# harman097/RoboRugby

Measured on AMD Instinct MI355X. Metric: env_steps_per_sec, higher is better.
Workload: dtype f64

## Files before the change

roborugby_amd/build.py:

```python
import hashlib
import os
import re
import shutil
import subprocess

HERE = os.path.dirname(os.path.abspath(__file__))
SRC = os.path.join(HERE, "csrc", "rr_kernels.hip")
SRC_KSTEP = os.path.join(HERE, "csrc", "rr_kstep_inst.hip")
SRC_DQN = os.path.join(HERE, "csrc", "rr_dqn.hip")
HDR_KSTEP = os.path.join(HERE, "csrc", "rr_kstep.hpp")
DEPS = [SRC, SRC_KSTEP, SRC_DQN, HDR_KSTEP, os.path.join(HERE, "csrc", "rr_sim.hpp"),
        os.path.join(HERE, "csrc", "rr_extras.hpp"), os.path.join(HERE, "csrc", "rr_hive.hpp"),
        os.path.join(os.path.dirname(HERE), "include", "roborugby_amd.h")]
LIB = os.path.join(HERE, "libroborugby_amd.so")
LIB_EXACT = os.path.join(HERE, "libroborugby_amd_exact.so")
HIPCC_FLAGS = ["-O3", "--offload-arch=gfx950", "-std=c++17", "-ffp-contract=off", "-fPIC", "-shared"]


def header_config_table():
    with open(HDR_KSTEP) as f:
        text = f.read()
    parts = int(re.search(r"^#define RR_KSTEP_PARTS (\d+)$", text, re.M).group(1))
    table = re.search(r"^#else // the product library.*?^#endif", text, re.M | re.S).group(0)
    rows = [tuple(int(v) for v in m.groups()) for m in re.finditer(r"X\((\d+), (\d+), (\d+), (\d+), (\d+), (\d+), \w+, \d+, [01]\)", table)]
    if not rows or sorted({r[1] for r in rows}) != list(range(parts)):
        raise RuntimeError("csrc/rr_kstep.hpp: the configuration table does not use every part 0..RR_KSTEP_PARTS-1")
    return parts, {r[2:] for r in rows}


KSTEP_PARTS = 7
BUILT_SHAPES = {(1, 0, 1, 0), (2, 2, 4, 4), (1, 1, 1, 1)}


def find_hipcc():
    for cand in (shutil.which("hipcc"), "/opt/rocm/bin/hipcc"):
        if cand and os.path.exists(cand):
            return cand
    raise RuntimeError("hipcc not found: the MI355X library cannot be built here")


def sources_present():
    return all(os.path.exists(d) for d in DEPS)


def source_hash():
    h = hashlib.sha256(" ".join(HIPCC_FLAGS).encode())
    for d in DEPS:
        with open(d, "rb") as f:
            h.update(os.path.basename(d).encode() + b"\0" + f.read())
    return h.hexdigest()


def is_stale(exact=False):
    lib = LIB_EXACT if exact else LIB
    if not os.path.exists(lib) or not os.path.exists(lib + ".srchash"):
        return True
    with open(lib + ".srchash") as f:
        return f.read().strip() != source_hash()


def build_hip_library(force=False, verbose=False, jobs=None, exact=False):
    lib_path = LIB_EXACT if exact else LIB
    if not force and not is_stale(exact):
        return lib_path
    import tempfile
    from concurrent.futures import ThreadPoolExecutor
    if header_config_table() != (KSTEP_PARTS, BUILT_SHAPES):
        raise RuntimeError("roborugby_amd/build.py: KSTEP_PARTS / BUILT_SHAPES differ from the table in csrc/rr_kstep.hpp")
    digest = source_hash()
    hipcc = find_hipcc()
    cflags = [f for f in HIPCC_FLAGS if f != "-shared"] + (["-DRR_EXACT_TRIG=1"] if exact else [])
    jobs = jobs or int(os.environ.get("RR_BUILD_JOBS", "0")) or min(8, os.cpu_count() or 1)
    with tempfile.TemporaryDirectory(prefix="rr_build_") as tmpd:
        units = [(SRC, ["-DRR_SPLIT_BUILD"], os.path.join(tmpd, "rr_kernels.o"))]
        units += [(SRC_KSTEP, [f"-DRR_PART={k}"], os.path.join(tmpd, f"rr_kstep_{k}.o")) for k in range(KSTEP_PARTS)]
        units += [(SRC_DQN, [], os.path.join(tmpd, "rr_dqn.o"))]

        def compile_one(u):
            src, defs, obj = u
            cmd = [hipcc] + cflags + defs + ["-c", "-o", obj, src]
            if verbose:
                print(" ".join(cmd), flush=True)
            subprocess.check_call(cmd)
            return obj

        with ThreadPoolExecutor(max_workers=jobs) as ex:
            objs = list(ex.map(compile_one, units))
        tmp = lib_path + f".tmp{os.getpid()}"
        cmd = [hipcc, "--offload-arch=gfx950", "-fPIC", "-shared", "-o", tmp] + objs
        if verbose:
            print(" ".join(cmd), flush=True)
        subprocess.check_call(cmd)
    os.replace(tmp, lib_path)
    with open(lib_path + ".srchash", "w") as f:
# ... 61 lines not shown
```

roborugby_amd/csrc/rr_kernels.hip:

```cpp
#include <hip/hip_runtime.h>
#include <stdio.h>
#include <string.h>
#include <cmath>
#include <new>
#include <string>
#include <type_traits>
#include <cstdlib>

#include "../../include/roborugby_amd.h"
#include "rr_sim.hpp"
#include "rr_extras.hpp"
#include "rr_hive.hpp"
#include "rr_kstep.hpp"

using namespace rr;


#ifndef RR_ORDER_SHIFT
#define RR_ORDER_SHIFT 2
#endif
constexpr int ORDER_BINS = 1024, ORDER_THREADS = 1024;
__global__ __launch_bounds__(ORDER_THREADS) void k_order(const uint32_t *cost, uint32_t *order, int ngroups) {
    __shared__ uint32_t hist[ORDER_BINS];
    for (int i = threadIdx.x; i < ORDER_BINS; i += ORDER_THREADS) hist[i] = 0;
    __syncthreads();
    for (int g = threadIdx.x; g < ngroups; g += ORDER_THREADS) {
        uint32_t c = cost[g] >> RR_ORDER_SHIFT;
        c = c > ORDER_BINS - 1 ? ORDER_BINS - 1 : c;
        atomicAdd(&hist[ORDER_BINS - 1 - c], 1u);
    }
    __syncthreads();
    __shared__ uint32_t scan[ORDER_BINS];
    uint32_t v = hist[threadIdx.x];
    scan[threadIdx.x] = v;
    __syncthreads();
    for (int off = 1; off < ORDER_BINS; off <<= 1) {
        uint32_t add = threadIdx.x >= (unsigned)off ? scan[threadIdx.x - off] : 0u;
        __syncthreads();
        scan[threadIdx.x] += add;
        __syncthreads();
    }
    hist[threadIdx.x] = scan[threadIdx.x] - v;
    __syncthreads();
    for (int g = threadIdx.x; g < ngroups; g += ORDER_THREADS) {
        uint32_t c = cost[g] >> RR_ORDER_SHIFT;
        c = c > ORDER_BINS - 1 ? ORDER_BINS - 1 : c;
        order[atomicAdd(&hist[ORDER_BINS - 1 - c], 1u)] = (uint32_t)g;
    }
}
__global__ void k_iota(uint32_t *order, int n) {
    int i = blockIdx.x * blockDim.x + threadIdx.x;
    if (i < n) order[i] = (uint32_t)i;
}

template <class C, typename O>
__global__ __launch_bounds__(64 * WAVES_PER_BLOCK) void k_reset(SimParams<typename C::Real> sp, typename C::Store *recs,
                                                               int32_t *irecs, int n, const uint8_t *mask, int init,
                                                               O *obs, O *obs_g) {
    using R = typename C::Real;
    __shared__ Arena<C> lds[arenas_per_block<C>()];
    const int wave = threadIdx.x / C::VW;
    const int arena = blockIdx.x * arenas_per_block<C>() + wave;
    if (arena >= n || wave >= arenas_per_block<C>()) return;
    Arena<C> &A = lds[wave];
    typename C::Store *rec = recs + (size_t)arena * Arena<C>::P_STRIDE;
    int32_t *irec = irecs + (size_t)arena * Arena<C>::I_STRIDE;
    int st = 0;
    if (init) {
        const int lane = threadIdx.x & (C::VW - 1);
        R *p = reinterpret_cast<R *>(&A.p);
        int32_t *q = reinterpret_cast<int32_t *>(&A.i);
        for (int k = lane; k < Arena<C>::P_REALS; k += C::VW) p[k] = (R)0;
        for (int k = lane; k < Arena<C>::I_INTS; k += C::VW) q[k] = 0;
        RR_SYNC();
        if (lane < C::NR) robot_set_clean_lane(A, sp, lane, (R)0, (R)0, lane < C::NRH ? (R)90 : (R)-90);
        if (lane < C::NB) ball_set_clean_lane(A, lane, (R)0, (R)0, (R)0, (R)0);
        if (lane == 0) A.i.episode = -1;
        RR_SYNC();
    } else {
        load_record(A, rec, irec);
    }
    const bool doit = init || !mask || mask[arena];
    if (doit) reset_arena(A, sp, sp.arena_offset + (uint64_t)arena, (uint64_t)(uint32_t)(A.i.episode + 1), st);
    else derive(A, sp);
    if (obs && doit) observe<C, O>(A, sp, 1, -1, -1, obs + (size_t)arena * 11, st);
    if (obs_g && doit) {
        if (!observe<C, O>(A, sp, -1, -1, -1, obs_g + (size_t)arena * 11, st)) {
            for (int k = threadIdx.x & (C::VW - 1); k < 11; k += C::VW) obs_g[(size_t)arena * 11 + k] = (O)NAN;
        }
    }
    store_record(A, rec, irec);
}

template <class C, typename O>
__global__ __launch_bounds__(64 * WAVES_PER_BLOCK) void k_observe(SimParams<typename C::Real> sp, const typename C::Store *recs,
                                                                 const int32_t *irecs, int n, int team, int ridx, int bidx,
                                                                 O *obs) {
    __shared__ Arena<C> lds[arenas_per_block<C>()];
    const int wave = threadIdx.x / C::VW;
    const int arena = blockIdx.x * arenas_per_block<C>() + wave;
    if (arena >= n || wave >= arenas_per_block<C>()) return;
    Arena<C> &A = lds[wave];
    load_record(A, recs + (size_t)arena * Arena<C>::P_STRIDE, irecs + (size_t)arena * Arena<C>::I_STRIDE);
    derive(A, sp);
    int st = 0;
    if (!observe<C, O>(A, sp, team, ridx, bidx, obs + (size_t)arena * 11, st)) {
        for (int k = threadIdx.x & (C::VW - 1); k < 11; k += C::VW) obs[(size_t)arena * 11 + k] = (O)NAN;
    }
}

template <class C>
__global__ void k_set_state(typename C::Store *recs, int32_t *irecs, int n, const double *robots, const int32_t *ri,
                            const double *balls, const int32_t *step) {
    using R = typename C::Real;
    int a = blockIdx.x * blockDim.x + threadIdx.x;
    if (a >= n) return;
    typename C::Store *rec = recs + (size_t)a * Arena<C>::P_STRIDE;
    int32_t *irec = irecs + (size_t)a * Arena<C>::I_STRIDE;
    using L = RecLayout<C>;
    constexpr int NR = C::NR, NB = C::NB;
    for (int r = 0; r < NR; r++) {
        for (int f = 0; f < L::ROBOT_FIELDS; f++) rec[L::robot_field(f) + r] = (typename C::Store)robots[((size_t)a * NR + r) * L::ROBOT_FIELDS + f];
        for (int f = 0; f < 3; f++) irec[L::robot_int(f) + r] = ri[((size_t)a * NR + r) * 3 + f];
    }
    for (int b = 0; b < NB; b++)
        for (int f = 0; f < L::BALL_FIELDS; f++) rec[L::ball_field(f) + b] = (typename C::Store)balls[((size_t)a * NB + b) * L::BALL_FIELDS + f];
    irec[L::STEP] = step[a];
    irec[L::FAULT] = 0;
    irec[L::FZP] = 0;
#if RR_CARRY
    rec[L::IC] = rec[L::BCX + NB - 1]; rec[L::IC + 1] = rec[L::BCY + NB - 1];
#endif
// ... 123 lines not shown
    int a = blockIdx.x * blockDim.x + threadIdx.x;
    if (a >= n) return;
    if (record_parked<C>(irecs + (size_t)a * Arena<C>::I_STRIDE)) *flag = 1;
}
template <class C>
__global__ void k_goal_clear(int n, int32_t *gs, const uint8_t *mask) {
    int a = blockIdx.x * blockDim.x + threadIdx.x;
    if (a >= n || (mask && !mask[a])) return;
    goal_state_clear<C>(gs + (size_t)a * gs_stride<C>());
}
template <class C>
__global__ void k_goal_scores(int n, const int32_t *gs, int32_t *scores) {
    int a = blockIdx.x * blockDim.x + threadIdx.x;
    if (a >= n) return;
    for (int k = 0; k < 2; k++) scores[2 * a + k] = goal_score<C>(gs + (size_t)a * gs_stride<C>(), k);
}
template <class C, typename O>
__global__ void k_observe_kind(SimParams<typename C::Real> sp, const typename C::Store *recs, int n, int kind, int team, int ridx,
                               int bidx, O *obs, int dim, const typename C::Real *xs) {
    int a = blockIdx.x * blockDim.x + threadIdx.x;
    if (a >= n) return;
    Rec<C> q = { recs + (size_t)a * Arena<C>::P_STRIDE };
    O tmp[6 * C::NR + 4 * C::NB > 11 ? 6 * C::NR + 4 * C::NB : 11];
    const int m = observe_kind<C, O>(q, sp, kind, team, ridx, bidx, tmp, xs ? xs + (size_t)a * xs_stride<C>() : nullptr);
    for (int k = 0; k < dim; k++) obs[(size_t)a * dim + k] = k < m ? tmp[k] : (O)NAN;
}

template <class C, typename O, int KIND>
__global__ __launch_bounds__(64 * WAVES_PER_BLOCK, lds_waves_per_simd<C>()) void k_hive(SimParams<typename C::Real> sp, const typename C::Store *recs,
                                                              const int32_t *irecs, int n, uint32_t robot_mask, int32_t *assign,
                                                              O *obs) {
    __shared__ Arena<C> lds[arenas_per_block<C>()];
    const int wave = threadIdx.x / C::VW;
    const int arena = blockIdx.x * arenas_per_block<C>() + wave;
    if (arena >= n || wave >= arenas_per_block<C>()) return;
    Arena<C> &A = lds[wave];
    const typename C::Store *rec = recs + (size_t)arena * Arena<C>::P_STRIDE;
    load_record(A, rec, irecs + (size_t)arena * Arena<C>::I_STRIDE);
    if (KIND == OBS_V2) derive(A, sp);
    Rec<C> q = { rec };
    hive_observe<C, O, KIND>(A, q, sp, robot_mask, assign + (size_t)arena * C::NR, obs + (size_t)arena * C::NR * 11);
}

__global__ void k_policy_chase(const float *obs, int n, int na, uint32_t noise_u32, uint64_t seed, uint64_t arena_offset,
                               const int32_t *step_of, uint32_t step, int32_t *actions) {
    const int a = blockIdx.x * blockDim.x + threadIdx.x;
    if (a >= n) return;
    const float d = fmodf(obs[(size_t)a * 11 + 1] - obs[(size_t)a * 11 + 0] + 540.0f, 360.0f) - 180.0f;
    int act = fabsf(d) < 8.0f ? 0 : (d > 0.0f ? 2 : 3);
    const uint64_t gid = arena_offset + (uint64_t)a;
    const uint32_t st = step_of ? (uint32_t)step_of[a] : step;
    uint32_t c[4] = { (uint32_t)gid, (uint32_t)(gid >> 32), st, 0x70C1u };
    philox4x32(c, (uint32_t)seed, (uint32_t)(seed >> 32));
    if (c[0] < noise_u32) act = (int)(c[1] & 7u);
    actions[(size_t)a * na] = act;
    for (int k = 1; k < na; k++) actions[(size_t)a * na + k] = (int)((c[2 + (k & 1)] >> (4 * (k >> 1))) & 7u);
}

typedef unsigned int u32x4 __attribute__((ext_vector_type(4)));
__global__ __launch_bounds__(256) void k_copy16(const u32x4 *__restrict__ src, u32x4 *__restrict__ dst, size_t n16) {
    const size_t i = (size_t)blockIdx.x * 256 + threadIdx.x;
    if (i < n16) dst[i] = src[i];
}

struct rr_env {
    rr_config cfg;
    int kind;
    int vw;
    void *recs;
    int32_t *irecs;
    size_t rec_bytes, irec_bytes;
    uint32_t *snap;
    int32_t *isnap;
    SimParams<double> spd;
    SimParams<float> spf;
    Program prog;
    bool custom_prog;
    bool track_prior;
    int32_t *gs;
    void *xs;
    int32_t *status_buf;
    uint32_t *order;
    uint32_t *cost;
    int ngroups;
    uint32_t *park;
    uint32_t budget;
    int32_t *flag;
};

static thread_local std::string g_err;
static int fail(int code, const std::string &msg) { g_err = msg; return code; }
#define HIP_TRY(expr)                                                                            \
    do {                                                                                         \
        hipError_t e_ = (expr);                                                                  \
        if (e_ != hipSuccess) return fail(-2, std::string(#expr) + ": " + hipGetErrorString(e_)); \
    } while (0)

template <typename R> static void fill_params(SimParams<R> &sp, const rr_config &c) {
    derive_constants(sp, c.arena_w, c.arena_h);
    sp.game_len = c.game_len_steps; sp.game_mode = c.game_mode; sp.time_limit = c.time_limit; sp.auto_reset = c.auto_reset;
    sp.reset_on_fault = c.reset_on_fault;
    sp.acc_external = 0;
    { const char *nm = getenv("RR_NO_MEMO"); sp.memo = (nm && atoi(nm)) ? 0 : 1; }
    sp.seed = c.seed; sp.arena_offset = c.arena_offset;
}
template <typename R> static const SimParams<R> &params_of(const rr_env *e);
template <> const SimParams<double> &params_of<double>(const rr_env *e) { return e->spd; }
template <> const SimParams<float> &params_of<float>(const rr_env *e) { return e->spf; }

template <class F> static int dispatch(const rr_env *e, F &&f) {
#define X(kind_, part_, a, b, c, d, R_, vw_, def_) \
    if (e->kind == kind_ && e->vw == vw_) return f(Cfg<a, b, c, d, R_, vw_>{});
    RR_CFG_TABLE(X)
#undef X
    return fail(-1, "corrupt handle");
}
struct DeviceGuard {
    int prev = -1;
    bool switched = false;
    explicit DeviceGuard(int want) {
        if (hipGetDevice(&prev) == hipSuccess && prev != want) switched = (hipSetDevice(want) == hipSuccess);
    }
    ~DeviceGuard() { if (switched) (void)hipSetDevice(prev); }
};

template <class C> struct Typed {
    using Cfg = C;
    using R = typename C::Real;
    const rr_env *e;
    hipStream_t s;
    int n() const { return e->cfg.num_envs; }
    typename C::Store *recs() const { return static_cast<typename C::Store *>(e->recs); }
    int32_t *irecs() const { return e->irecs; }
    R *xs() const { return static_cast<R *>(e->xs); }
    const SimParams<R> &sp() const { return params_of<R>(e); }
    template <class... P, class... A> void per_thread(void (*k)(P...), const A &...a) const {
        hipLaunchKernelGGL(k, dim3((unsigned)((n() + 127) / 128)), dim3(128), 0, s, static_cast<P>(a)...);
    }
    template <class... P, class... A> void per_wave(void (*k)(P...), const A &...a) const {
        hipLaunchKernelGGL(k, dim3((unsigned)((n() + arenas_per_block<C>() - 1) / arenas_per_block<C>())), dim3(64 * WAVES_PER_BLOCK), 0, s,
                           static_cast<P>(a)...);
    }
};
template <typename O = float, class F>
static int on_handle(rr_env *e, const char *who, void *stream, F &&f, const char *f64_refusal = nullptr) {
    if (!e) return fail(-1, std::string(who) + ": null handle");
    DeviceGuard guard(e->cfg.device);
    int rc = dispatch(e, [&](auto c) {
        using C = decltype(c);
        if constexpr (std::is_same<O, double>::value && !std::is_same<typename C::Real, double>::value) return fail(-1, f64_refusal);
        else return f(Typed<C>{ e, (hipStream_t)stream });
    });
    if (rc) return rc;
    HIP_TRY(hipGetLastError());
    return 0;
}

extern "C" {

int rr_abi_version(void) { return RR_ABI_VERSION; }
int rr_exact_trig(void) { return RR_EXACT_TRIG; }
const char *rr_last_error(void) { return g_err.c_str(); }

int rr_create(const rr_config *cfg, rr_env **out) {
    if (!cfg || !out) return fail(-1, "rr_create: null argument");
    if (cfg->struct_size != (int32_t)sizeof(rr_config)) return fail(-1, "rr_create: rr_config.struct_size mismatch");
    if (cfg->num_envs <= 0) return fail(-1, "rr_create: num_envs must be positive");
    int shape = -1;
#define X(kind_, part_, a, b, c, d, R_, vw_, def_) \
    if (shape < 0 && cfg->nr_happy == a && cfg->nr_grumpy == b && cfg->nb_pos == c && cfg->nb_neg == d) shape = kind_ % RR_NUM_SHAPES;
    RR_CFG_TABLE(X)
#undef X
#if defined(RR_CUSTOM_SHAPE)
    if (shape < 0) return fail(-1, "rr_create: this library was built for one shape only (roborugby_amd.build.build_shape_library) and it is not this one");
    if (cfg->dtype == RR_DTYPE_F32) return fail(-1, "rr_create: a one-shape library is built for RR_DTYPE_F64 and RR_DTYPE_F32_STATE only");
#else
    if (shape < 0)
        return fail(-1, "rr_create: unsupported entity counts (built shapes: 1+0 robots/1+0 balls, 2+2 robots/4+4 balls, 1+1 robots/1+1 balls; "
                        "any other counts: a one-shape library, roborugby_amd.build.build_shape_library / BatchedRoboRugbyEnv does it on demand)");
#endif
    if (cfg->dtype != RR_DTYPE_F64 && cfg->dtype != RR_DTYPE_F32 && cfg->dtype != RR_DTYPE_F32_STATE) return fail(-1, "rr_create: bad dtype");
    if (cfg->dtype == RR_DTYPE_F32_STATE && cfg->step_budget_clocks) return fail(-1, "rr_create: no step budget with RR_DTYPE_F32_STATE");
    if (!(cfg->arena_w >= 300 && cfg->arena_h >= 300 && cfg->arena_w <= 8192 && cfg->arena_h <= 8192))
        return fail(-1, "rr_create: arena size out of range [300, 8192]");
    if (cfg->game_len_steps <= 0) return fail(-1, "rr_create: game_len_steps must be positive");
    int ndev = 0;
    HIP_TRY(hipGetDeviceCount(&ndev));
    if (cfg->device < 0 || cfg->device >= ndev) return fail(-1, "rr_create: no such HIP device");
    DeviceGuard guard(cfg->device);
    rr_env *e = new (std::nothrow) rr_env();
    if (!e) return fail(-3, "rr_create: out of host memory");
    e->cfg = *cfg;
    e->kind = shape + RR_NUM_SHAPES * cfg->dtype;
    e->prog.n = 3; e->prog.id[0] = KEEPER_NAUGHTY; e->prog.id[1] = KEEPER_CHASE; e->prog.id[2] = KEEPER_PUSHPOS;
    const char *want = getenv("RR_VW");
    const int want_vw = want ? atoi(want) : 0;
#define X(kind_, part_, a, b, c, d, R_, vw_, def_) \
    if (e->kind == kind_ && (e->vw == 0 || want_vw == vw_)) e->vw = vw_;
    RR_CFG_TABLE(X)
#undef X
    fill_params(e->spd, *cfg);
    fill_params(e->spf, *cfg);
    size_t pstride = 0, preals = 0, snapw = 0, isnapw = 0;
    int apb = 1;
    const size_t rsz = cfg->dtype == RR_DTYPE_F64 ? 8 : 4;
    dispatch(e, [&](auto c) {
        using CC = decltype(c);
        pstride = Arena<CC>::P_STRIDE; preals = Arena<CC>::P_REALS; snapw = Arena<CC>::SNAP_WORDS; isnapw = Arena<CC>::ISNAP_WORDS;
        apb = arenas_per_block<CC>();
        return 0;
    });
    const int n = cfg->num_envs;
    e->rec_bytes = pstride * rsz;
    e->irec_bytes = 0;
    hipError_t he = hipMalloc(&e->recs, e->rec_bytes * (size_t)n);
    if (he == hipSuccess && e->spd.memo) {
        he = hipMalloc((void **)&e->snap, 4 * snapw * (size_t)n);
        if (he == hipSuccess) he = hipMalloc((void **)&e->isnap, 4 * isnapw * (size_t)n);
    }
    if (he != hipSuccess) {
        rr_destroy(e);
        return fail(-3, std::string("rr_create: hipMalloc: ") + hipGetErrorString(he));
    }
    e->irecs = reinterpret_cast<int32_t *>(static_cast<char *>(e->recs) + preals * rsz);
    const int ng = (n + apb - 1) / apb;
    const char *no = getenv("RR_NO_ORDER");
    if (ng > 2048 && ng <= 65536 && !(no && atoi(no))) {
        if (hipMalloc((void **)&e->order, sizeof(uint32_t) * ng) == hipSuccess && hipMalloc((void **)&e->cost, sizeof(uint32_t) * ng) == hipSuccess) {
            e->ngroups = ng;
            hipLaunchKernelGGL(k_iota, dim3((ng + 255) / 256), dim3(256), 0, 0, e->order, ng);
            (void)hipMemset(e->cost, 0, sizeof(uint32_t) * ng);
        } else {
            if (e->order) (void)hipFree(e->order);
            e->order = nullptr; e->cost = nullptr;
        }
    }
    dispatch(e, [&](auto c) {
        Typed<decltype(c)> v = { e, nullptr };
        v.per_wave(k_reset<decltype(c), float>, v.sp(), v.recs(), v.irecs(), n, nullptr, 1, nullptr, nullptr);
        return 0;
    });
    he = hipGetLastError();
    if (he == hipSuccess) he = hipDeviceSynchronize();
    if (he != hipSuccess) {
        rr_destroy(e);
        return fail(-2, std::string("rr_create: init kernel: ") + hipGetErrorString(he));
    }
    if (cfg->step_budget_clocks) {
        if (int rc = rr_set_step_budget(e, cfg->step_budget_clocks)) { rr_destroy(e); return rc; }
    }
    *out = e;
    return 0;
}

int rr_destroy(rr_env *e) {
    if (!e) return 0;
    DeviceGuard guard(e->cfg.device);
    for (void *p : { e->recs, (void *)e->snap, (void *)e->isnap, e->xs, (void *)e->gs, (void *)e->status_buf, (void *)e->order, (void *)e->cost,
                     (void *)e->park, (void *)e->flag })
        if (p) (void)hipFree(p);
    delete e;
    return 0;
}

int rr_reset(rr_env *e, const uint8_t *mask, float *obs, float *obs_g, void *stream) {
    return on_handle(e, "rr_reset", stream, [&](auto v) {
        using C = typename decltype(v)::Cfg;
        v.per_wave(k_reset<C, float>, v.sp(), v.recs(), v.irecs(), v.n(), mask, 0, obs, obs_g);
        if (e->track_prior && e->xs)
            v.per_thread(k_extras_begin<C>, v.recs(), v.n(), v.xs(), mask);
        if (e->gs) v.per_thread(k_goal_clear<C>, v.n(), e->gs, mask);
        return 0;
    });
}

static int check_step_args(rr_env *e, const void *act, int32_t na, const void *obs, const void *reward, const void *done) {
    if (!e) return fail(-1, "rr_step: null handle");
    if (!act || !obs || !reward || !done) return fail(-1, "rr_step: actions/obs/reward/done must be non-null");
    const int nr = e->cfg.nr_happy + e->cfg.nr_grumpy;
    if (na < 0 || na > nr)
        return fail(-1, "rr_step: more actions than robots");
    return 0;
}

extern "C++" {
template <typename O>
static int step_impl(rr_env *e, const int32_t *actions, const float *thrust, int32_t na, O *obs, O *reward, uint8_t *done,
                     O *obs_g, O *reward_g, int32_t *status, void *stream, int nsteps = 1, int repeat = 0) {
    if ((e->custom_prog || e->track_prior || e->gs) && !status) status = e->status_buf;
    return on_handle<O>(e, "rr_step", stream, [&](auto v) {
        using C = typename decltype(v)::Cfg;
        const int n = v.n();
        const bool extras = e->custom_prog || e->track_prior;
        auto step = [&](auto kernel, int ns, int rep, uint32_t *park, uint32_t budget) {
            v.per_wave(kernel, v.sp(), v.recs(), v.irecs(), n, actions, thrust, na, obs, reward, done, obs_g, reward_g, status, e->order, e->cost,
                       ns, rep, e->snap, e->isnap, park, budget);
        };
        if (extras) v.per_thread(k_extras_begin<C>, v.recs(), n, v.xs(), nullptr);
        if constexpr (C::MIXED) {
            if (nsteps != 1 || e->park) return fail(-1, "RR_DTYPE_F32_STATE: rr_step only (no rr_rollout, no step budget)");
            step(k_step<C, O, false>, 1, 0, nullptr, 0);
        } else {
            if (nsteps == 1 && e->park) step(k_step<C, O, false, true>, 1, 0, e->park, e->budget);
            else if (nsteps == 1) step(k_step<C, O, false>, 1, 0, nullptr, 0);
            else if constexpr (std::is_same<O, float>::value && default_width<C>()) step(k_step<C, O, true>, nsteps, repeat, nullptr, 0);
            else return fail(-1, "rr_rollout: built for float outputs and the default lane widths (RR_VW unset) only");
        }
        if (e->order) hipLaunchKernelGGL(k_order, dim3(1), dim3(ORDER_THREADS), 0, v.s, (const uint32_t *)e->cost, e->order, e->ngroups);
        if (extras) v.per_thread(k_extras_end<C, O>, v.sp(), v.recs(), n, v.xs(), e->prog, e->custom_prog ? 1 : 0, reward, reward_g, status, done);
        if (e->gs) {
            int bd = 0;
            for (int k = 0; k < e->prog.n; k++) bd |= e->prog.id[k] == KEEPER_BASEDESTRUCTION;
            v.per_thread(k_goal<C, O>, v.sp(), v.recs(), v.irecs(), n, e->gs, bd, reward, reward_g, done, status);
        }
        return 0;
    }, "fp64 outputs need a handle created with RR_DTYPE_F64");
}
}

int rr_step(rr_env *e, const int32_t *actions, int32_t na, float *obs, float *reward, uint8_t *done, float *obs_g,
            float *reward_g, int32_t *status, void *stream) {
    if (int rc = check_step_args(e, actions, na, obs, reward, done)) return rc;
    return step_impl<float>(e, actions, nullptr, na, obs, reward, done, obs_g, reward_g, status, stream);
}
int rr_rollout(rr_env *e, const int32_t *actions, int32_t na, int32_t nsteps, int32_t repeat, float *obs, float *reward,
               uint8_t *done, float *obs_g, float *reward_g, int32_t *status, void *stream) {
    if (int rc = check_step_args(e, actions, na, obs, reward, done)) return rc;
    if (nsteps < 1 || nsteps > 4096) return fail(-1, "rr_rollout: nsteps must be in 1..4096");
    if (e->custom_prog || e->track_prior || e->gs)
        return fail(-1, "rr_rollout: the side kernels of a custom reward program / prior-step tracking / goal scoring bracket single steps; use rr_step");
    if (e->park) return fail(-1, "rr_rollout: not on a handle that has had a step budget (arenas may be parked mid-step); use rr_step");
    return step_impl<float>(e, actions, nullptr, na, obs, reward, done, obs_g, reward_g, status, stream, (int)nsteps, repeat != 0);
}
int rr_step_thrust(rr_env *e, const float *thrust, int32_t nk, float *obs, float *reward, uint8_t *done, float *obs_g,
                   float *reward_g, int32_t *status, void *stream) {
    if (int rc = check_step_args(e, thrust, nk, obs, reward, done)) return rc;
    return step_impl<float>(e, nullptr, thrust, nk, obs, reward, done, obs_g, reward_g, status, stream);
}
int rr_step_f64(rr_env *e, const int32_t *actions, int32_t na, double *obs, double *reward, uint8_t *done, double *obs_g,
                double *reward_g, int32_t *status, void *stream) {
    if (int rc = check_step_args(e, actions, na, obs, reward, done)) return rc;
    return step_impl<double>(e, actions, nullptr, na, obs, reward, done, obs_g, reward_g, status, stream);
}
int rr_step_thrust_f64(rr_env *e, const float *thrust, int32_t nk, double *obs, double *reward, uint8_t *done, double *obs_g,
                       double *reward_g, int32_t *status, void *stream) {
    if (int rc = check_step_args(e, thrust, nk, obs, reward, done)) return rc;
    return step_impl<double>(e, nullptr, thrust, nk, obs, reward, done, obs_g, reward_g, status, stream);
}

static int ensure_snapshot_buffer(rr_env *e) {
    if (e->xs) return 0;
    size_t bytes = 0;
    dispatch(e, [&](auto c) { using C = decltype(c); bytes = sizeof(typename C::Real) * xs_stride<C>() * (size_t)e->cfg.num_envs; return 0; });
    HIP_TRY(hipMalloc(&e->xs, bytes));
    HIP_TRY(hipMemset(e->xs, 0, bytes));
    return 0;
}
static int ensure_status_buffer(rr_env *e) {
    if (!e->status_buf) HIP_TRY(hipMalloc((void **)&e->status_buf, sizeof(int32_t) * (size_t)e->cfg.num_envs));
    return 0;
}

static int any_parked(rr_env *e, void *stream, bool &parked) {
    parked = false;
    if (!e->park) return 0;
    hipStream_t s = (hipStream_t)stream;
    if (!e->flag) HIP_TRY(hipMalloc((void **)&e->flag, sizeof(int32_t)));
    HIP_TRY(hipMemsetAsync(e->flag, 0, sizeof(int32_t), s));
    if (int rc = on_handle(e, "any_parked", stream, [&](auto v) {
            v.per_thread(k_any_parked<typename decltype(v)::Cfg>, v.irecs(), v.n(), e->flag);
            return 0;
        }))
        return rc;
    int32_t h = 0;
    HIP_TRY(hipMemcpyAsync(&h, e->flag, sizeof(int32_t), hipMemcpyDeviceToHost, s));
    HIP_TRY(hipStreamSynchronize(s));
    parked = h != 0;
    return 0;
}
static int refuse_if_parked_without_copies(rr_env *e, void *stream, const char *who) {
    if (e->custom_prog || e->track_prior || !e->park) return 0;
    bool parked = false;
    if (int rc = any_parked(e, stream, parked)) return rc;
    if (parked)
        return fail(-1, std::string(who) + ": arenas are parked mid-step (budgeted step) and no on_step_begin copies were kept when their "
                                           "step began; rr_set_step_budget(env, 0) and one rr_step complete every parked step first");
    return 0;
}

int rr_set_reward_program(rr_env *e, const int32_t *ids, int32_t n) {
    if (!e || (!ids && n > 0)) return fail(-1, "rr_set_reward_program: null argument");
// ... 260 lines not shown
```

roborugby_amd/csrc/rr_kstep.hpp:

```cpp
#pragma once
#include <hip/hip_runtime.h>
#include <stdint.h>
#include <type_traits>
#include "rr_sim.hpp"

using namespace rr;

template <class C> __device__ __forceinline__ void load_record(Arena<C> &A, const typename C::Store *rec, const int32_t *irec) {
    using R = typename C::Real;
    R *p = reinterpret_cast<R *>(&A.p);
    int32_t *q = reinterpret_cast<int32_t *>(&A.i);
    const int lane = threadIdx.x & (C::VW - 1);
    for (int k = lane; k < Arena<C>::P_REALS; k += C::VW) p[k] = (R)rec[k];
    for (int k = lane; k < Arena<C>::I_INTS; k += C::VW) q[k] = irec[k];
    RR_SYNC();
}
template <class C> __device__ __forceinline__ void store_record(const Arena<C> &A, typename C::Store *rec, int32_t *irec) {
    using R = typename C::Real;
    const R *p = reinterpret_cast<const R *>(&A.p);
    const int32_t *q = reinterpret_cast<const int32_t *>(&A.i);
    const int lane = threadIdx.x & (C::VW - 1);
    RR_SYNC();
    for (int k = lane; k < Arena<C>::P_REALS; k += C::VW) rec[k] = (typename C::Store)p[k];
    constexpr int TAIL = Arena<C>::I_STRIDE - Arena<C>::P_REALS * Arena<C>::WS;
    for (int k = lane; k < TAIL; k += C::VW) irec[k] = k < Arena<C>::I_INTS ? q[k] : 0;
}

#ifndef RR_MIN_WAVES_PER_SIMD
#define RR_MIN_WAVES_PER_SIMD 4
#endif
#ifndef RR_WAVES_PER_BLOCK
#define RR_WAVES_PER_BLOCK 1
#endif
constexpr int WAVES_PER_BLOCK = RR_WAVES_PER_BLOCK;
#ifdef RR_ARENAS_PER_WAVE
template <class C> constexpr int arenas_per_block() { return (C::VW == 8 ? RR_ARENAS_PER_WAVE : 64 / C::VW) * WAVES_PER_BLOCK; }
#else
template <class C> constexpr int arenas_per_block() { return 64 * WAVES_PER_BLOCK / C::VW; }
#endif
template <class C> constexpr int lds_waves_per_simd() {
#ifdef RR_FORCE_WAVES
    return RR_FORCE_WAVES;
#endif
    constexpr int per_cu = (160 * 1024) / (int)(sizeof(Arena<C>) * arenas_per_block<C>()) * WAVES_PER_BLOCK;
    return per_cu / 4 < 1 ? 1 : (per_cu / 4 > RR_MIN_WAVES_PER_SIMD ? RR_MIN_WAVES_PER_SIMD : per_cu / 4);
}


template <class C, typename O, bool MULTI, bool BUDGET = false>
__global__ __launch_bounds__(64 * WAVES_PER_BLOCK, lds_waves_per_simd<C>()) void k_step(SimParams<typename C::Real> sp, typename C::Store *recs,
                                                              int32_t *irecs, int n, const int32_t *actions,
                                                              const float *thrust, int na, O *obs, O *reward,
                                                              uint8_t *done, O *obs_g, O *reward_g, int32_t *status,
                                                              const uint32_t *order, uint32_t *cost, int nsteps, int repeat,
                                                              uint32_t *snap, int32_t *isnap, uint32_t *park = nullptr,
                                                              uint32_t budget = 0) {
    static_assert(!(MULTI && BUDGET), "rr_rollout keeps the record in LDS across steps: no barrier to budget");
#ifdef RR_FAKE_LDS_ARENAS
    __shared__ Arena<C> lds[RR_FAKE_LDS_ARENAS];
#else
    __shared__ Arena<C> lds[arenas_per_block<C>()];
#endif
    const int wave = threadIdx.x / C::VW;
#ifdef RR_ARENAS_PER_WAVE
    if (wave >= arenas_per_block<C>()) return;
#endif
    const unsigned long long t_begin = (cost || BUDGET) ? __builtin_amdgcn_s_memtime() : 0ull;
    const int group = order ? (int)order[blockIdx.x] : (int)blockIdx.x;
    const int arena = group * arenas_per_block<C>() + wave;
    if (arena >= n) return;
    Arena<C> &A = lds[wave];
    typename C::Store *rec = recs + (size_t)arena * Arena<C>::P_STRIDE;
    int32_t *irec = irecs + (size_t)arena * Arena<C>::I_STRIDE;
    RR_T0();
#if defined(RR_PROFILE_PHASES)
    const unsigned long long rr_wave_t0_ = __builtin_amdgcn_s_memrealtime();
#endif
    load_record(A, rec, irec);
    derive(A, sp);
    RR_STAMP(12);
    if constexpr (!MULTI) {
        StepOut<O> o = { obs, obs_g, reward, reward_g, done, status, sp.memo ? snap : nullptr, isnap, arena,
                         (int)Arena<C>::SNAP_WORDS, (int)Arena<C>::ISNAP_WORDS };
        if constexpr (BUDGET) {
            ParkCtx pk;
            pk.buf = park + (size_t)arena * Arena<C>::PARK_WORDS; pk.budget = budget; pk.t_begin = t_begin;
            step_arena<C, O, true>(A, sp, sp.arena_offset + (uint64_t)arena, actions ? actions + (size_t)arena * na : nullptr,
                                   thrust ? thrust + (size_t)arena * 2 * na : nullptr, na, o, pk);
        } else {
            step_arena<C, O>(A, sp, sp.arena_offset + (uint64_t)arena, actions ? actions + (size_t)arena * na : nullptr,
                             thrust ? thrust + (size_t)arena * 2 * na : nullptr, na, o);
        }
    } else {
#pragma unroll 1
        for (int s = 0; s < nsteps; s++) {
            const size_t so = (size_t)s * (size_t)n;
            StepOut<O> o = { obs + so * 11, obs_g ? obs_g + so * 11 : nullptr, reward + so, reward_g ? reward_g + so : nullptr, done + so,
                             status ? status + so : nullptr, sp.memo ? snap : nullptr, isnap, arena,
                             (int)Arena<C>::SNAP_WORDS, (int)Arena<C>::ISNAP_WORDS };
            const size_t ao = repeat ? 0 : so;
            step_arena<C, O>(A, sp, sp.arena_offset + (uint64_t)arena, actions ? actions + (ao + (size_t)arena) * na : nullptr,
                             thrust ? thrust + (ao + (size_t)arena) * 2 * na : nullptr, na, o);
        }
    }
    RR_TR();
    {
        int arena_again = arena;
        asm volatile("" : "+v"(arena_again));
        store_record(A, recs + (size_t)arena_again * Arena<C>::P_STRIDE, irecs + (size_t)arena_again * Arena<C>::I_STRIDE);
    }
    RR_STAMP(13);
    if (cost && threadIdx.x == 0) {
        const unsigned long long dt = ((__builtin_amdgcn_s_memtime() - t_begin) >> 8) / (unsigned)(MULTI ? nsteps : 1);
        cost[group] = dt > 0xFFFFull ? 0xFFFFu : (uint32_t)dt;
    }
#if defined(RR_PROFILE_PHASES)
    if ((threadIdx.x & 63) == 0 && blockIdx.x < 65536) {
        g_rr_wave_t[2 * blockIdx.x] = rr_wave_t0_;
        g_rr_wave_t[2 * blockIdx.x + 1] = __builtin_amdgcn_s_memrealtime();
    }
#endif
}

#define RR_KSTEP_PARTS 7
#if defined(RR_CUSTOM_SHAPE)
#define RR_CFG_TABLE(X) X(0, 0, RR_NRH, RR_NRG, RR_NBP, RR_NBN, double, RR_CVW, 1) X(6, 0, RR_NRH, RR_NRG, RR_NBP, RR_NBN, F32State, RR_CVW, 1)
#elif defined(RR_CFG_SUBSET) && RR_CFG_SUBSET == 2
#define RR_CFG_TABLE(X) X(0, 0, 1, 0, 1, 0, double, 4, 0) X(1, 0, 2, 2, 4, 4, double, 8, 1)
#elif defined(RR_CFG_SUBSET) && RR_CFG_SUBSET == 3
#define RR_CFG_TABLE(X) X(2, 0, 1, 1, 1, 1, double, 4, 1) X(1, 0, 2, 2, 4, 4, double, 8, 1)
#elif defined(RR_CFG_SUBSET)
#define RR_CFG_TABLE(X) X(0, 0, 1, 0, 1, 0, double, 2, 1) X(1, 0, 2, 2, 4, 4, double, 8, 1)
#else
#define RR_CFG_TABLE(X)                                                                                                                    \
    X(0, 5, 1, 0, 1, 0, double, 2, 1) X(0, 5, 1, 0, 1, 0, double, 4, 0) X(0, 6, 1, 0, 1, 0, double, 8, 0) X(0, 6, 1, 0, 1, 0, double, 64, 0)     \
    X(1, 0, 2, 2, 4, 4, double, 8, 1) X(1, 1, 2, 2, 4, 4, double, 16, 0) X(1, 2, 2, 2, 4, 4, double, 32, 0) X(1, 3, 2, 2, 4, 4, double, 64, 0)   \
    X(2, 1, 1, 1, 1, 1, double, 4, 1) X(2, 2, 1, 1, 1, 1, double, 8, 0) X(2, 3, 1, 1, 1, 1, double, 64, 0)                                    \
    X(3, 6, 1, 0, 1, 0, float, 2, 1) X(3, 6, 1, 0, 1, 0, float, 4, 0) X(3, 6, 1, 0, 1, 0, float, 64, 0)                                       \
    X(4, 4, 2, 2, 4, 4, float, 8, 1) X(4, 4, 2, 2, 4, 4, float, 16, 0) X(4, 5, 2, 2, 4, 4, float, 64, 0)                                      \
    X(5, 0, 1, 1, 1, 1, float, 4, 1)                                                                                                      \
    X(6, 5, 1, 0, 1, 0, F32State, 2, 1) X(7, 2, 2, 2, 4, 4, F32State, 8, 1) X(8, 6, 1, 1, 1, 1, F32State, 4, 1)
#endif
constexpr int RR_NUM_SHAPES = 3;
#define X(kind_, part_, a, b, c, d, R_, vw_, def_) static_assert(part_ >= 0 && part_ < RR_KSTEP_PARTS && kind_ >= 0 && kind_ < 3 * RR_NUM_SHAPES, "row");
RR_CFG_TABLE(X)
#undef X
template <class C> constexpr bool default_width() {
#define X(kind_, part_, a, b, c, d, R_, vw_, def_) if (std::is_same<C, Cfg<a, b, c, d, R_, vw_>>::value) return def_ != 0;
    RR_CFG_TABLE(X)
#undef X
    return false;
}

#define RR_KSTEP_SIG(C_, O_)                                                                                                       \
    (SimParams<typename C_::Real>, typename C_::Store *, int32_t *, int, const int32_t *, const float *, int, O_ *, O_ *, uint8_t *, \
     O_ *, O_ *, int32_t *, const uint32_t *, uint32_t *, int, int, uint32_t *, int32_t *, uint32_t *, uint32_t)
#define RR_KSTEP_CFG(a, b, c, d, R_, vw_) Cfg<a, b, c, d, R_, vw_>
#define RR_KSTEP_ONE(PREFIX, a, b, c, d, R_, vw_, O_, MULTI_, BUDGET_) \
    PREFIX template __global__ void k_step<Cfg<a, b, c, d, R_, vw_>, O_, MULTI_, BUDGET_> RR_KSTEP_SIG(RR_KSTEP_CFG(a, b, c, d, R_, vw_), O_);
#define RR_KSTEP_PLAIN(PREFIX, a, b, c, d, R_, vw_, O_) RR_KSTEP_ONE(PREFIX, a, b, c, d, R_, vw_, O_, false, false)
#define RR_KSTEP_MULTI_0(PREFIX, a, b, c, d, R_, vw_, O_)
#define RR_KSTEP_MULTI_1(PREFIX, a, b, c, d, R_, vw_, O_) RR_KSTEP_ONE(PREFIX, a, b, c, d, R_, vw_, O_, true, false)
#define RR_KSTEP_VARIANTS(PREFIX, a, b, c, d, R_, vw_, O_, MULTI_) \
    RR_KSTEP_PLAIN(PREFIX, a, b, c, d, R_, vw_, O_) RR_KSTEP_ONE(PREFIX, a, b, c, d, R_, vw_, O_, false, true) RR_KSTEP_MULTI_##MULTI_(PREFIX, a, b, c, d, R_, vw_, O_)
#define RR_KSTEP_INST_double(PREFIX, a, b, c, d, vw_, def_) \
    RR_KSTEP_VARIANTS(PREFIX, a, b, c, d, double, vw_, float, def_) RR_KSTEP_VARIANTS(PREFIX, a, b, c, d, double, vw_, double, 0)
#define RR_KSTEP_INST_float(PREFIX, a, b, c, d, vw_, def_) RR_KSTEP_VARIANTS(PREFIX, a, b, c, d, float, vw_, float, def_)
#define RR_KSTEP_INST_F32State(PREFIX, a, b, c, d, vw_, def_) \
    RR_KSTEP_PLAIN(PREFIX, a, b, c, d, F32State, vw_, float) RR_KSTEP_PLAIN(PREFIX, a, b, c, d, F32State, vw_, double)

#if defined(RR_SPLIT_BUILD) && !defined(RR_CFG_SUBSET)
#define X(kind_, part_, a, b, c, d, R_, vw_, def_) RR_KSTEP_INST_##R_(extern, a, b, c, d, vw_, def_)
RR_CFG_TABLE(X)
#undef X
#endif
```

Measured before the change: 174.0 million.

## Fold cost-order sort into step kernel block zero with double-buffered order arrays

Removes the separate single-block k_order launch after each step. Block 0 of the step kernel now sorts the previous call's costs into the alternate order buffer using a one-wave, multi-pass LDS histogram, while the other blocks simulate using the current order. The intent is to drop a serialized kernel launch and its tail from the step loop. In exchange, the ordering lags by one call and the sort runs on a single wave inside the step kernel.

Measured after the change: 173.9 million. About the same (-0.1%).

```diff
diff --git a/roborugby_amd/build.py b/roborugby_amd/build.py
--- a/roborugby_amd/build.py
+++ b/roborugby_amd/build.py
@@ -9,7 +9,7 @@
 SRC_KSTEP = os.path.join(HERE, "csrc", "rr_kstep_inst.hip")
 SRC_DQN = os.path.join(HERE, "csrc", "rr_dqn.hip")
 HDR_KSTEP = os.path.join(HERE, "csrc", "rr_kstep.hpp")
-DEPS = [SRC, SRC_KSTEP, SRC_DQN, HDR_KSTEP, os.path.join(HERE, "csrc", "rr_sim.hpp"),
+DEPS = [SRC, SRC_KSTEP, SRC_DQN, HDR_KSTEP, os.path.join(HERE, "csrc", "rr_sim.hpp"), os.path.join(HERE, "csrc", "rr_order.hpp"),
         os.path.join(HERE, "csrc", "rr_extras.hpp"), os.path.join(HERE, "csrc", "rr_hive.hpp"),
         os.path.join(os.path.dirname(HERE), "include", "roborugby_amd.h")]
 LIB = os.path.join(HERE, "libroborugby_amd.so")
diff --git a/roborugby_amd/csrc/rr_kernels.hip b/roborugby_amd/csrc/rr_kernels.hip
--- a/roborugby_amd/csrc/rr_kernels.hip
+++ b/roborugby_amd/csrc/rr_kernels.hip
@@ -16,38 +16,6 @@
 using namespace rr;
 
 
-#ifndef RR_ORDER_SHIFT
-#define RR_ORDER_SHIFT 2
-#endif
-constexpr int ORDER_BINS = 1024, ORDER_THREADS = 1024;
-__global__ __launch_bounds__(ORDER_THREADS) void k_order(const uint32_t *cost, uint32_t *order, int ngroups) {
-    __shared__ uint32_t hist[ORDER_BINS];
-    for (int i = threadIdx.x; i < ORDER_BINS; i += ORDER_THREADS) hist[i] = 0;
-    __syncthreads();
-    for (int g = threadIdx.x; g < ngroups; g += ORDER_THREADS) {
-        uint32_t c = cost[g] >> RR_ORDER_SHIFT;
-        c = c > ORDER_BINS - 1 ? ORDER_BINS - 1 : c;
-        atomicAdd(&hist[ORDER_BINS - 1 - c], 1u);
-    }
-    __syncthreads();
-    __shared__ uint32_t scan[ORDER_BINS];
-    uint32_t v = hist[threadIdx.x];
-    scan[threadIdx.x] = v;
-    __syncthreads();
-    for (int off = 1; off < ORDER_BINS; off <<= 1) {
-        uint32_t add = threadIdx.x >= (unsigned)off ? scan[threadIdx.x - off] : 0u;
-        __syncthreads();
-        scan[threadIdx.x] += add;
-        __syncthreads();
-    }
-    hist[threadIdx.x] = scan[threadIdx.x] - v;
-    __syncthreads();
-    for (int g = threadIdx.x; g < ngroups; g += ORDER_THREADS) {
-        uint32_t c = cost[g] >> RR_ORDER_SHIFT;
-        c = c > ORDER_BINS - 1 ? ORDER_BINS - 1 : c;
-        order[atomicAdd(&hist[ORDER_BINS - 1 - c], 1u)] = (uint32_t)g;
-    }
-}
 __global__ void k_iota(uint32_t *order, int n) {
     int i = blockIdx.x * blockDim.x + threadIdx.x;
     if (i < n) order[i] = (uint32_t)i;
@@ -337,6 +305,7 @@
     int32_t *status_buf;
     uint32_t *order;
     uint32_t *cost;
+    int cur;
     int ngroups;
     uint32_t *park;
     uint32_t budget;
@@ -392,8 +361,9 @@
     template <class... P, class... A> void per_thread(void (*k)(P...), const A &...a) const {
         hipLaunchKernelGGL(k, dim3((unsigned)((n() + 127) / 128)), dim3(128), 0, s, static_cast<P>(a)...);
     }
-    template <class... P, class... A> void per_wave(void (*k)(P...), const A &...a) const {
-        hipLaunchKernelGGL(k, dim3((unsigned)((n() + arenas_per_block<C>() - 1) / arenas_per_block<C>())), dim3(64 * WAVES_PER_BLOCK), 0, s,
+    template <class... P, class... A> void per_wave(void (*k)(P...), const A &...a) const { waves(0, k, a...); }
+    template <class... P, class... A> void waves(unsigned extra, void (*k)(P...), const A &...a) const {
+        hipLaunchKernelGGL(k, dim3(extra + (unsigned)((n() + arenas_per_block<C>() - 1) / arenas_per_block<C>())), dim3(64 * WAVES_PER_BLOCK), 0, s,
                            static_cast<P>(a)...);
     }
 };
@@ -481,10 +451,10 @@
     const int ng = (n + apb - 1) / apb;
     const char *no = getenv("RR_NO_ORDER");
     if (ng > 2048 && ng <= 65536 && !(no && atoi(no))) {
-        if (hipMalloc((void **)&e->order, sizeof(uint32_t) * ng) == hipSuccess && hipMalloc((void **)&e->cost, sizeof(uint32_t) * ng) == hipSuccess) {
+        if (hipMalloc((void **)&e->order, sizeof(uint32_t) * 2 * ng) == hipSuccess && hipMalloc((void **)&e->cost, sizeof(uint32_t) * 2 * ng) == hipSuccess) {
             e->ngroups = ng;
-            hipLaunchKernelGGL(k_iota, dim3((ng + 255) / 256), dim3(256), 0, 0, e->order, ng);
-            (void)hipMemset(e->cost, 0, sizeof(uint32_t) * ng);
+            for (int k = 0; k < 2; k++) hipLaunchKernelGGL(k_iota, dim3((ng + 255) / 256), dim3(256), 0, 0, e->order + (size_t)k * ng, ng);
+            (void)hipMemset(e->cost, 0, sizeof(uint32_t) * 2 * ng);
         } else {
             if (e->order) (void)hipFree(e->order);
             e->order = nullptr; e->cost = nullptr;
@@ -548,8 +518,10 @@
         const int n = v.n();
         const bool extras = e->custom_prog || e->track_prior;
         auto step = [&](auto kernel, int ns, int rep, uint32_t *park, uint32_t budget) {
-            v.per_wave(kernel, v.sp(), v.recs(), v.irecs(), n, actions, thrust, na, obs, reward, done, obs_g, reward_g, status, e->order, e->cost,
-                       ns, rep, e->snap, e->isnap, park, budget);
+            const size_t at = e->order ? (size_t)e->cur * e->ngroups : 0;
+            v.waves(e->order ? 1 : 0, kernel, v.sp(), v.recs(), v.irecs(), n, actions, thrust, na, obs, reward, done, obs_g, reward_g, status,
+                    e->order + at, e->cost + at, e->cur ? -e->ngroups : e->ngroups, ns, rep, e->snap, e->isnap, park, budget);
+            e->cur ^= 1;
         };
         if (extras) v.per_thread(k_extras_begin<C>, v.recs(), n, v.xs(), nullptr);
         if constexpr (C::MIXED) {
@@ -561,7 +533,6 @@
             else if constexpr (std::is_same<O, float>::value && default_width<C>()) step(k_step<C, O, true>, nsteps, repeat, nullptr, 0);
             else return fail(-1, "rr_rollout: built for float outputs and the default lane widths (RR_VW unset) only");
         }
-        if (e->order) hipLaunchKernelGGL(k_order, dim3(1), dim3(ORDER_THREADS), 0, v.s, (const uint32_t *)e->cost, e->order, e->ngroups);
         if (extras) v.per_thread(k_extras_end<C, O>, v.sp(), v.recs(), n, v.xs(), e->prog, e->custom_prog ? 1 : 0, reward, reward_g, status, done);
         if (e->gs) {
             int bd = 0;
diff --git a/roborugby_amd/csrc/rr_kstep.hpp b/roborugby_amd/csrc/rr_kstep.hpp
--- a/roborugby_amd/csrc/rr_kstep.hpp
+++ b/roborugby_amd/csrc/rr_kstep.hpp
@@ -3,6 +3,7 @@
 #include <stdint.h>
 #include <type_traits>
 #include "rr_sim.hpp"
+#include "rr_order.hpp"
 
 using namespace rr;
 
@@ -45,6 +46,11 @@
     constexpr int per_cu = (160 * 1024) / (int)(sizeof(Arena<C>) * arenas_per_block<C>()) * WAVES_PER_BLOCK;
     return per_cu / 4 < 1 ? 1 : (per_cu / 4 > RR_MIN_WAVES_PER_SIMD ? RR_MIN_WAVES_PER_SIMD : per_cu / 4);
 }
+constexpr int order_pass_bins(size_t lds_bytes) {
+    int b = 64;
+    while (b < ORDER_BINS && (size_t)b * 2 * sizeof(uint32_t) <= lds_bytes) b *= 2;
+    return b;
+}
 
 
 template <class C, typename O, bool MULTI, bool BUDGET = false>
@@ -52,7 +58,7 @@
                                                               int32_t *irecs, int n, const int32_t *actions,
                                                               const float *thrust, int na, O *obs, O *reward,
                                                               uint8_t *done, O *obs_g, O *reward_g, int32_t *status,
-                                                              const uint32_t *order, uint32_t *cost, int nsteps, int repeat,
+                                                              const uint32_t *order, uint32_t *cost, int other, int nsteps, int repeat,
                                                               uint32_t *snap, int32_t *isnap, uint32_t *park = nullptr,
                                                               uint32_t budget = 0) {
     static_assert(!(MULTI && BUDGET), "rr_rollout keeps the record in LDS across steps: no barrier to budget");
@@ -61,12 +67,24 @@
 #else
     __shared__ Arena<C> lds[arenas_per_block<C>()];
 #endif
+    if (__builtin_expect(blockIdx.x == 0, 0) && order) {
+        if (threadIdx.x >= 64) return;
+#if defined(RR_PROFILE_PHASES)
+        const unsigned long long rr_sort_t0_ = __builtin_amdgcn_s_memrealtime();
+#endif
+        order_sort<order_pass_bins(sizeof(lds))>(cost + other, const_cast<uint32_t *>(order) + other, other < 0 ? -other : other,
+                                                 (RR_ORD_LDS uint32_t *)&lds[0]);
+#if defined(RR_PROFILE_PHASES)
+        if (threadIdx.x == 0) { g_rr_wave_t[0] = rr_sort_t0_; g_rr_wave_t[1] = __builtin_amdgcn_s_memrealtime(); }
+#endif
+        return;
+    }
     const int wave = threadIdx.x / C::VW;
 #ifdef RR_ARENAS_PER_WAVE
     if (wave >= arenas_per_block<C>()) return;
 #endif
     const unsigned long long t_begin = (cost || BUDGET) ? __builtin_amdgcn_s_memtime() : 0ull;
-    const int group = order ? (int)order[blockIdx.x] : (int)blockIdx.x;
+    const int group = order ? (int)order[blockIdx.x - 1] : (int)blockIdx.x;
     const int arena = group * arenas_per_block<C>() + wave;
     if (arena >= n) return;
     Arena<C> &A = lds[wave];
@@ -154,7 +172,7 @@
 
 #define RR_KSTEP_SIG(C_, O_)                                                                                                       \
     (SimParams<typename C_::Real>, typename C_::Store *, int32_t *, int, const int32_t *, const float *, int, O_ *, O_ *, uint8_t *, \
-     O_ *, O_ *, int32_t *, const uint32_t *, uint32_t *, int, int, uint32_t *, int32_t *, uint32_t *, uint32_t)
+     O_ *, O_ *, int32_t *, const uint32_t *, uint32_t *, int, int, int, uint32_t *, int32_t *, uint32_t *, uint32_t)
 #define RR_KSTEP_CFG(a, b, c, d, R_, vw_) Cfg<a, b, c, d, R_, vw_>
 #define RR_KSTEP_ONE(PREFIX, a, b, c, d, R_, vw_, O_, MULTI_, BUDGET_) \
     PREFIX template __global__ void k_step<Cfg<a, b, c, d, R_, vw_>, O_, MULTI_, BUDGET_> RR_KSTEP_SIG(RR_KSTEP_CFG(a, b, c, d, R_, vw_), O_);
diff --git a/roborugby_amd/csrc/rr_order.hpp b/roborugby_amd/csrc/rr_order.hpp
--- /dev/null
+++ b/roborugby_amd/csrc/rr_order.hpp
@@ -0,0 +1,102 @@
+#pragma once
+#include <stdint.h>
+
+#ifndef RR_ORDER_SHIFT
+#define RR_ORDER_SHIFT 2
+#endif
+
+#if defined(__HIPCC__) && defined(__HIP_DEVICE_COMPILE__)
+#define RR_ORD_FOR_LANES(l) for (int l = (int)(threadIdx.x & 63), l##_o = 0; l##_o < 1; ++l##_o)
+#define RR_ORD_SYNC()                                                \
+    do {                                                             \
+        __builtin_amdgcn_fence(__ATOMIC_RELEASE, "wavefront");       \
+        __builtin_amdgcn_wave_barrier();                             \
+        __builtin_amdgcn_fence(__ATOMIC_ACQUIRE, "wavefront");       \
+    } while (0)
+#define RR_ORD_VAR(type, name) type name
+#define RR_ORD_V(name, l) name
+#define RR_ORD_UP(name, l, off) ((uint32_t)__shfl_up((int)(name), (unsigned)(off), 64))
+#define RR_ORD_LAST(name) ((uint32_t)__shfl((int)(name), 63, 64))
+#define RR_ORD_BUMP(p) __hip_atomic_fetch_add(p, 1u, __ATOMIC_RELAXED, __HIP_MEMORY_SCOPE_WORKGROUP)
+#define RR_ORD_LDS __attribute__((address_space(3)))
+#else
+#define RR_ORD_FOR_LANES(l) for (int l = 0; l < 64; ++l)
+#define RR_ORD_SYNC() do { } while (0)
+#define RR_ORD_VAR(type, name) type name[64]
+#define RR_ORD_V(name, l) name[l]
+#define RR_ORD_UP(name, l, off) name[(l) >= (off) ? (l) - (off) : (l)]
+#define RR_ORD_LAST(name) name[63]
+#define RR_ORD_BUMP(p) ((*(p))++)
+#define RR_ORD_LDS
+#endif
+#if defined(__HIPCC__)
+#define RR_ORD_FN __device__ __forceinline__
+#else
+#define RR_ORD_FN inline
+#endif
+
+namespace rr {
+
+constexpr int ORDER_BINS = 1024;
+constexpr int ORDER_BATCH = 8;
+
+RR_ORD_FN int order_bin(uint32_t cost) {
+    const uint32_t c = cost >> RR_ORDER_SHIFT;
+    return ORDER_BINS - 1 - (int)(c > ORDER_BINS - 1 ? ORDER_BINS - 1 : c);
+}
+
+template <int PASS_BINS>
+RR_ORD_FN void order_sort(const uint32_t *cost, uint32_t *order, int ng, RR_ORD_LDS uint32_t *hist) {
+    static_assert(PASS_BINS >= 64 && PASS_BINS <= ORDER_BINS && (PASS_BINS & (PASS_BINS - 1)) == 0, "a power of two, a bin per lane at least");
+    constexpr int K = PASS_BINS / 64;
+    uint32_t placed = 0;
+    for (int lo = 0; lo < ORDER_BINS && placed < (uint32_t)ng; lo += PASS_BINS) {
+        RR_ORD_FOR_LANES(l) for (int i = l; i < PASS_BINS; i += 64) hist[i] = 0;
+        RR_ORD_SYNC();
+        RR_ORD_FOR_LANES(l) for (int g0 = l; g0 < ng; g0 += 64 * ORDER_BATCH) {
+            uint32_t c[ORDER_BATCH];
+#pragma unroll
+            for (int j = 0; j < ORDER_BATCH; j++) c[j] = g0 + 64 * j < ng ? cost[g0 + 64 * j] : 0u;
+#pragma unroll
+            for (int j = 0; j < ORDER_BATCH; j++) {
+                const unsigned b = (unsigned)(order_bin(c[j]) - lo);
+                if (g0 + 64 * j < ng && b < (unsigned)PASS_BINS) (void)RR_ORD_BUMP(&hist[b]);
+            }
+        }
+        RR_ORD_SYNC();
+        RR_ORD_VAR(uint32_t, tot);
+        RR_ORD_VAR(uint32_t, incl);
+        RR_ORD_VAR(uint32_t, up);
+        RR_ORD_FOR_LANES(l) {
+            uint32_t s = 0;
+            for (int k = 0; k < K; k++) { const uint32_t v = hist[l * K + k]; hist[l * K + k] = s; s += v; }
+            RR_ORD_V(tot, l) = RR_ORD_V(incl, l) = s;
+        }
+        for (int off = 1; off < 64; off <<= 1) {
+            RR_ORD_FOR_LANES(l) RR_ORD_V(up, l) = RR_ORD_UP(incl, l, off);
+            RR_ORD_FOR_LANES(l) if (l >= off) RR_ORD_V(incl, l) += RR_ORD_V(up, l);
+        }
+        RR_ORD_FOR_LANES(l) {
+            const uint32_t first = placed + RR_ORD_V(incl, l) - RR_ORD_V(tot, l);
+            for (int k = 0; k < K; k++) hist[l * K + k] += first;
+        }
+        placed += RR_ORD_LAST(incl);
+        RR_ORD_SYNC();
+        RR_ORD_FOR_LANES(l) for (int g0 = l; g0 < ng; g0 += 64 * ORDER_BATCH) {
+            uint32_t c[ORDER_BATCH];
+#pragma unroll
+            for (int j = 0; j < ORDER_BATCH; j++) c[j] = g0 + 64 * j < ng ? cost[g0 + 64 * j] : 0u;
+#pragma unroll
+            for (int j = 0; j < ORDER_BATCH; j++) {
+                const unsigned b = (unsigned)(order_bin(c[j]) - lo);
+                if (g0 + 64 * j < ng && b < (unsigned)PASS_BINS) {
+                    const uint32_t at = RR_ORD_BUMP(&hist[b]);
+                    if (at < (uint32_t)ng) order[at] = (uint32_t)(g0 + 64 * j);
+                }
+            }
+        }
+        RR_ORD_SYNC();
+    }
+}
+
+}
```
